# MichSchli/RelationPrediction

Measured on NVIDIA H100. Metric: R-GCN layer fwd+bwd M-edges/sec, higher is better.
Workload: dtype f32

## Files before the change

relationprediction_b200/csrc/gemm_tf32x3.cu:

```cuda
#include <cuda_runtime.h>
#include <stdint.h>

#include <algorithm>
#include <cstdlib>

#include "kernels.cuh"

namespace {

constexpr int BM = 128, BN = 128, BK = 32;
constexpr int STAGES = 3;
constexpr int TILE_BYTES = BM * BK * 4;
constexpr int STAGE_BYTES = 4 * TILE_BYTES;
constexpr int SMEM_BYTES = STAGES * STAGE_BYTES + 1024;
constexpr int N_PRODUCERS = 128;
constexpr int N_CONSUMERS = 256;
constexpr int N_THREADS = N_PRODUCERS + N_CONSUMERS;
constexpr int N_FRAG = BN / 2;
static_assert(BM == BN, "the producers use one row schedule for both operands");

__device__ __forceinline__ uint32_t smem_u32(const void* p) {
  return (uint32_t)__cvta_generic_to_shared(p);
}
__device__ __forceinline__ void mbar_init(uint64_t* bar, uint32_t count) {
  asm volatile("mbarrier.init.shared::cta.b64 [%0], %1;" ::"r"(smem_u32(bar)), "r"(count));
}
__device__ __forceinline__ void mbar_arrive(uint64_t* bar) {
  asm volatile("mbarrier.arrive.shared::cta.b64 _, [%0];" ::"r"(smem_u32(bar)) : "memory");
}
__device__ __forceinline__ void mbar_wait(uint64_t* bar, uint32_t parity) {
  asm volatile(
      "{\n\t"
      ".reg .pred p;\n\t"
      "WAIT_LOOP:\n\t"
      "mbarrier.try_wait.parity.shared::cta.b64 p, [%0], %1;\n\t"
      "@p bra WAIT_DONE;\n\t"
      "bra WAIT_LOOP;\n\t"
      "WAIT_DONE:\n\t"
      "}" ::"r"(smem_u32(bar)),
      "r"(parity)
      : "memory");
}
__device__ __forceinline__ void cp_async16(uint32_t dst, const void* src, uint32_t src_bytes) {
  asm volatile("cp.async.cg.shared.global [%0], [%1], 16, %2;" ::"r"(dst), "l"(src), "r"(src_bytes)
               : "memory");
}

__device__ __forceinline__ uint64_t make_desc(uint32_t smem_addr) {
  return (uint64_t)((smem_addr & 0x3FFFFu) >> 4) | (1ull << 16) | ((uint64_t)(1024 >> 4) << 32) | (1ull << 62);
}

__device__ __forceinline__ void wgmma_tf32(float (&d)[N_FRAG], uint64_t da, uint64_t db, uint32_t accumulate) {
  asm volatile(
      "{\n\t"
      ".reg .pred p;\n\t"
      "setp.ne.b32 p, %66, 0;\n\t"
      "wgmma.mma_async.sync.aligned.m64n128k8.f32.tf32.tf32 "
      "{%0, %1, %2, %3, %4, %5, %6, %7, %8, %9, %10, %11, %12, %13, %14, %15, %16, %17, %18, %19, %20, %21, %22, "
      "%23, %24, %25, %26, %27, %28, %29, %30, %31, %32, %33, %34, %35, %36, %37, %38, %39, %40, %41, %42, %43, %44, "
      "%45, %46, %47, %48, %49, %50, %51, %52, %53, %54, %55, %56, %57, %58, %59, %60, %61, %62, %63}, "
      "%64, %65, p, 1, 1;\n\t"
      "}"
      : "+f"(d[0]), "+f"(d[1]), "+f"(d[2]), "+f"(d[3]), "+f"(d[4]), "+f"(d[5]), "+f"(d[6]), "+f"(d[7]),
        "+f"(d[8]), "+f"(d[9]), "+f"(d[10]), "+f"(d[11]), "+f"(d[12]), "+f"(d[13]), "+f"(d[14]), "+f"(d[15]),
        "+f"(d[16]), "+f"(d[17]), "+f"(d[18]), "+f"(d[19]), "+f"(d[20]), "+f"(d[21]), "+f"(d[22]), "+f"(d[23]),
        "+f"(d[24]), "+f"(d[25]), "+f"(d[26]), "+f"(d[27]), "+f"(d[28]), "+f"(d[29]), "+f"(d[30]), "+f"(d[31]),
        "+f"(d[32]), "+f"(d[33]), "+f"(d[34]), "+f"(d[35]), "+f"(d[36]), "+f"(d[37]), "+f"(d[38]), "+f"(d[39]),
        "+f"(d[40]), "+f"(d[41]), "+f"(d[42]), "+f"(d[43]), "+f"(d[44]), "+f"(d[45]), "+f"(d[46]), "+f"(d[47]),
        "+f"(d[48]), "+f"(d[49]), "+f"(d[50]), "+f"(d[51]), "+f"(d[52]), "+f"(d[53]), "+f"(d[54]), "+f"(d[55]),
        "+f"(d[56]), "+f"(d[57]), "+f"(d[58]), "+f"(d[59]), "+f"(d[60]), "+f"(d[61]), "+f"(d[62]), "+f"(d[63])
      : "l"(da), "l"(db), "r"(accumulate)
      : "memory");
}
__device__ __forceinline__ void fence_acc(float (&d)[N_FRAG]) {
#pragma unroll
  for (int i = 0; i < N_FRAG; ++i) asm volatile("" : "+f"(d[i])::"memory");
}

__device__ __forceinline__ void split_tf32_trunc(float a, float& hi, float& lo) {
  hi = __uint_as_float(__float_as_uint(a) & 0xffffe000u);
  lo = __uint_as_float(__float_as_uint(a - hi) & 0xffffe000u);
}
__device__ __forceinline__ void split_tf32(float a, float& hi, float& lo) {
  uint32_t h, l;
  asm("cvt.rna.tf32.f32 %0, %1;" : "=r"(h) : "f"(a));
  hi = __uint_as_float(h);
  asm("cvt.rna.tf32.f32 %0, %1;" : "=r"(l) : "f"(a - hi));
  lo = __uint_as_float(l);
}

__device__ __forceinline__ uint32_t swz(int r, int c) {
  return (uint32_t)((r >> 3) * 1024 + (r & 7) * 128 + ((c ^ (r & 7)) << 4));
}

__device__ __forceinline__ void init_barriers(uint64_t* full_bar, uint64_t* empty_bar) {
  for (int s = 0; s < STAGES; ++s) {
    mbar_init(&full_bar[s], N_PRODUCERS);
    mbar_init(&empty_bar[s], N_CONSUMERS);
  }
  asm volatile("fence.mbarrier_init.release.cluster;" ::: "memory");
}

__device__ __forceinline__ void consume_tile(uint32_t smem_base, uint64_t* full_bar, uint64_t* empty_bar, int g0,
                                             int num_kb, uint32_t a_rows, float (&big)[N_FRAG],
                                             float (&small)[N_FRAG]) {
  for (int kb = 0; kb < num_kb; ++kb) {
    const int g = g0 + kb;
    const int s = g % STAGES;
    mbar_wait(&full_bar[s], (uint32_t)(g / STAGES) & 1u);
    const uint32_t a_hi = smem_base + s * STAGE_BYTES + a_rows, a_lo = a_hi + TILE_BYTES;
    const uint32_t b_hi = smem_base + s * STAGE_BYTES + 2 * TILE_BYTES, b_lo = b_hi + TILE_BYTES;
    asm volatile("wgmma.fence.sync.aligned;" ::: "memory");
#pragma unroll
    for (int kk = 0; kk < BK / 8; ++kk) {
      const uint64_t dah = make_desc(a_hi + kk * 32), dal = make_desc(a_lo + kk * 32);
      const uint64_t dbh = make_desc(b_hi + kk * 32), dbl = make_desc(b_lo + kk * 32);
      const uint32_t acc = (kb == 0 && kk == 0) ? 0u : 1u;
      wgmma_tf32(small, dal, dbh, acc);
      wgmma_tf32(small, dah, dbl, 1u);
      wgmma_tf32(big, dah, dbh, acc);
    }
    asm volatile("wgmma.commit_group.sync.aligned;" ::: "memory");
    asm volatile("wgmma.wait_group.sync.aligned 0;" ::: "memory");
    fence_acc(big);
    fence_acc(small);
    mbar_arrive(&empty_bar[s]);
  }
}

struct RankEpi {
  const float* gold_sig;
  const int32_t* gold_col;
  const uint32_t* known;
  int words;
  int32_t* raw_cnt;
  int32_t* known_cnt;
};
__device__ __forceinline__ float sigmoid_ref(float x) { return 1.0f / (1.0f + expf(-x)); }

template <int EPI>
__global__ void __launch_bounds__(N_THREADS, 1)
    k_gemm_tf32x3(const float* __restrict__ A, int64_t lda, const float* __restrict__ Bhi,
                  const float* __restrict__ Blo, int64_t ldb, float* __restrict__ C, int64_t ldc,
                  int M, int N, int K, int accumulate, int n_tiles, RankEpi re) {
  extern __shared__ uint8_t smem_raw[];
  __shared__ __align__(8) uint64_t full_bar[STAGES], empty_bar[STAGES];

  const uint32_t smem_base = (smem_u32(smem_raw) + 1023u) & ~1023u;
  const int tid = threadIdx.x, lane = tid & 31;
  const int tn = (N + BN - 1) / BN;
  const int num_kb = (K + BK - 1) / BK;
  const int n_mine = (n_tiles - (int)blockIdx.x + (int)gridDim.x - 1) / (int)gridDim.x;
  const int total_g = n_mine * num_kb;

  if (tid == 0) init_barriers(full_bar, empty_bar);
  __syncthreads();

  if (tid < N_PRODUCERS) {
    const int c = tid & 7;
    const int rbase = tid >> 3;
    const uint32_t soff = swz(rbase, c);
    constexpr int NR = BM / 16;

    int b_kb = 0, b_tile = (int)blockIdx.x, b_stage = 0;
    size_t b_off = 0;
    uint32_t b_ok = 0;
    auto b_set_tile = [&]() {
      const int r0 = (b_tile % tn) * BN + rbase;
      b_ok = 0;
#pragma unroll
      for (int i = 0; i < NR; ++i) b_ok |= (r0 + 16 * i < N ? 1u : 0u) << i;
      b_off = (b_ok & 1u) ? (size_t)r0 * ldb + c * 4 : 0;
    };
    b_set_tile();
    auto issue_b = [&]() {
      const uint32_t b_hi = smem_base + b_stage * STAGE_BYTES + 2 * TILE_BYTES + soff, b_lo = b_hi + TILE_BYTES;
      const bool col_ok = b_kb * BK + c * 4 < K;
      const size_t kof = b_off + (size_t)b_kb * BK;
#pragma unroll
      for (int i = 0; i < NR; ++i) {
        const bool ok = col_ok && ((b_ok >> i) & 1u);
        const size_t o = kof + (size_t)(16 * i) * ldb;
        cp_async16(b_hi + 2048 * i, ok ? Bhi + o : Bhi, ok ? 16u : 0u);
        cp_async16(b_lo + 2048 * i, ok ? Blo + o : Blo, ok ? 16u : 0u);
      }
      asm volatile("cp.async.commit_group;" ::: "memory");
      b_stage = b_stage + 1 == STAGES ? 0 : b_stage + 1;
      if (++b_kb == num_kb) {
        b_kb = 0;
        b_tile += (int)gridDim.x;
        b_set_tile();
      }
    };
    int a_kb = 0, a_tile = (int)blockIdx.x;
    size_t a_off = 0;
    uint32_t a_ok = 0;
    auto a_set_tile = [&]() {
      const int r0 = (a_tile / tn) * BM + rbase;
      a_ok = 0;
#pragma unroll
      for (int i = 0; i < NR; ++i) a_ok |= (r0 + 16 * i < M ? 1u : 0u) << i;
      a_off = (a_ok & 1u) ? (size_t)r0 * lda + c * 4 : 0;
    };
    a_set_tile();
    auto load_a = [&](float4 (&v)[NR]) {
      const bool col_ok = a_kb * BK + c * 4 < K;
      const float* p = A + a_off + (size_t)a_kb * BK;
#pragma unroll
      for (int i = 0; i < NR; ++i)
        v[i] = (col_ok && ((a_ok >> i) & 1u)) ? __ldg(reinterpret_cast<const float4*>(p + (size_t)(16 * i) * lda))
                                               : make_float4(0.f, 0.f, 0.f, 0.f);
      if (++a_kb == num_kb) {
        a_kb = 0;
        a_tile += (int)gridDim.x;
        a_set_tile();
      }
    };
    constexpr int PF = 2;
    float4 vbuf[PF + 1][NR];
    mbar_wait(&empty_bar[0], 1u);
    issue_b();
    for (int p = 0; p < PF; ++p)
      if (p < total_g) load_a(vbuf[p]);
    int s = 0;
    uint32_t ph_next = 0;
    for (int g0 = 0; g0 < total_g; g0 += PF + 1) {
#pragma unroll
      for (int u = 0; u <= PF; ++u) {
        const int g = g0 + u;
        if (g >= total_g) break;
        const bool more = g + 1 < total_g;
        const int s1 = s + 1 == STAGES ? 0 : s + 1;
        if (s1 == 0) ph_next ^= 1u;
        if (more) {
          mbar_wait(&empty_bar[s1], ph_next ^ 1u);
          issue_b();
        }
        if (g + PF < total_g) load_a(vbuf[(u + PF) % (PF + 1)]);
        const uint32_t a_hi = smem_base + s * STAGE_BYTES + soff, a_lo = a_hi + TILE_BYTES;
#pragma unroll
        for (int i = 0; i < NR; ++i) {
          float4 hi, lo;
          split_tf32_trunc(vbuf[u][i].x, hi.x, lo.x);
          split_tf32_trunc(vbuf[u][i].y, hi.y, lo.y);
          split_tf32_trunc(vbuf[u][i].z, hi.z, lo.z);
          split_tf32_trunc(vbuf[u][i].w, hi.w, lo.w);
          asm volatile("st.shared.v4.f32 [%0], {%1, %2, %3, %4};" ::"r"(a_hi + 2048 * i), "f"(hi.x), "f"(hi.y),
                       "f"(hi.z), "f"(hi.w)
                       : "memory");
          asm volatile("st.shared.v4.f32 [%0], {%1, %2, %3, %4};" ::"r"(a_lo + 2048 * i), "f"(lo.x), "f"(lo.y),
                       "f"(lo.z), "f"(lo.w)
                       : "memory");
        }
        if (more)
          asm volatile("cp.async.wait_group 1;" ::: "memory");
        else
          asm volatile("cp.async.wait_group 0;" ::: "memory");
        asm volatile("fence.proxy.async.shared::cta;" ::: "memory");
        mbar_arrive(&full_bar[s]);
        s = s1;
      }
    }
  } else {
    const int ctid = tid - N_PRODUCERS;
    const int wg = ctid >> 7;
    const uint32_t a_rows = (uint32_t)(wg * 64 * 128);
    float big[N_FRAG], small[N_FRAG];
    for (int ti = 0; ti < n_mine; ++ti) {
      const int tile = (int)blockIdx.x + ti * (int)gridDim.x;
      const int m0 = (tile / tn) * BM, n0 = (tile % tn) * BN;
      consume_tile(smem_base, full_bar, empty_bar, ti * num_kb, num_kb, a_rows, big, small);
      const int r0 = m0 + wg * 64 + ((ctid >> 5) & 3) * 16 + (lane >> 2);
      const int c0 = n0 + 2 * (lane & 3);
#pragma unroll
      for (int h = 0; h < 2; ++h) {
        const int row = r0 + 8 * h;
        if (EPI == 1) {
          int raw = 0, kn = 0;
          if (row < M) {
            const float gold_s = __ldg(re.gold_sig + row);
            const int gold_c = __ldg(re.gold_col + row);
#pragma unroll
            for (int cb = 0; cb < BN / 32; ++cb) {
              const int chunk = n0 + 32 * cb;
              const uint32_t kw =
                  (re.known && chunk < N) ? __ldg(re.known + (size_t)row * re.words + (chunk >> 5)) : 0u;
#pragma unroll
              for (int jj = 0; jj < 4; ++jj) {
                const int j = 4 * cb + jj;
#pragma unroll
                for (int e = 0; e < 2; ++e) {
                  const int col = c0 + 8 * j + e;
                  const float v = big[4 * j + 2 * h + e] + small[4 * j + 2 * h + e];
                  if (col < N && (sigmoid_ref(v) >= gold_s || col == gold_c)) {
                    ++raw;
                    kn += (int)((kw >> (col & 31)) & 1u);
                  }
                }
              }
            }
          }
          raw += __shfl_xor_sync(0xffffffffu, raw, 1);
          raw += __shfl_xor_sync(0xffffffffu, raw, 2);
          kn += __shfl_xor_sync(0xffffffffu, kn, 1);
          kn += __shfl_xor_sync(0xffffffffu, kn, 2);
          if ((lane & 3) == 0 && row < M) {
            if (raw) atomicAdd(re.raw_cnt + row, raw);
            if (kn) atomicAdd(re.known_cnt + row, kn);
          }
          continue;
        }
        if (row >= M) continue;
        float* crow = C + (size_t)row * ldc;
#pragma unroll
        for (int j = 0; j < BN / 8; ++j) {
          const int col = c0 + 8 * j;
          if (col < N) {
            float2 o = make_float2(big[4 * j + 2 * h] + small[4 * j + 2 * h],
                                   big[4 * j + 2 * h + 1] + small[4 * j + 2 * h + 1]);
            if (accumulate) {
              const float2 old = *reinterpret_cast<const float2*>(crow + col);
              o.x += old.x;
              o.y += old.y;
            }
            *reinterpret_cast<float2*>(crow + col) = o;
          }
        }
      }
    }
  }
}

__global__ void __launch_bounds__(N_THREADS, 1)
    k_gemm_tn_tf32x3(const float* __restrict__ A, int64_t lda, const float* __restrict__ B, int64_t ldb,
                     float* __restrict__ C, int64_t ldc, int M, int N, int K, int kb_per_split) {
  extern __shared__ uint8_t smem_raw[];
  __shared__ __align__(8) uint64_t full_bar[STAGES], empty_bar[STAGES];
  const uint32_t smem_base = (smem_u32(smem_raw) + 1023u) & ~1023u;
  const int tid = threadIdx.x, warp = tid >> 5, lane = tid & 31;
  const int m0 = blockIdx.x * BM, n0 = blockIdx.y * BN;
  const int kb_total = (K + BK - 1) / BK;
  const int kb_begin = blockIdx.z * kb_per_split;
  const int num_kb = min(kb_per_split, kb_total - kb_begin);
  if (num_kb <= 0) return;

  if (tid == 0) init_barriers(full_bar, empty_bar);
  __syncthreads();

  if (tid < N_PRODUCERS) {
    constexpr int NC = 8;
    const int kr = (lane & 15) + 16 * (warp & 1);
    const int cm0 = (lane >> 4) + 16 * (warp >> 1);
    auto load_ab = [&](int kbi, float4 (&va)[NC], float4 (&vb)[NC]) {
      const int krow = (kb_begin + kbi) * BK + kr;
      const bool kok = krow < K;
      const float* pa = A + (size_t)(kok ? krow : 0) * lda + m0;
      const float* pb = B + (size_t)(kok ? krow : 0) * ldb + n0;
#pragma unroll
      for (int i = 0; i < NC; ++i) {
        const int cm = cm0 + 2 * i;
        va[i] = (kok && m0 + 4 * cm < M) ? __ldg(reinterpret_cast<const float4*>(pa + 4 * cm))
                                         : make_float4(0.f, 0.f, 0.f, 0.f);
        vb[i] = (kok && n0 + 4 * cm < N) ? __ldg(reinterpret_cast<const float4*>(pb + 4 * cm))
                                         : make_float4(0.f, 0.f, 0.f, 0.f);
      }
    };
    auto store4 = [&](uint32_t hi_base, const float4& v, int cm) {
      const float x[4] = {v.x, v.y, v.z, v.w};
#pragma unroll
      for (int j = 0; j < 4; ++j) {
        const int r = 4 * cm + j;
        const uint32_t off =
            (uint32_t)((r >> 3) * 1024 + (r & 7) * 128 + ((((kr >> 2) ^ (r & 7)) << 4) | ((kr & 3) << 2)));
        float hi, lo;
        split_tf32_trunc(x[j], hi, lo);
        asm volatile("st.shared.f32 [%0], %1;" ::"r"(hi_base + off), "f"(hi) : "memory");
        asm volatile("st.shared.f32 [%0], %1;" ::"r"(hi_base + TILE_BYTES + off), "f"(lo) : "memory");
      }
    };
    float4 va[2][NC], vb[2][NC];
    load_ab(0, va[0], vb[0]);
    for (int kb0 = 0; kb0 < num_kb; kb0 += 2) {
#pragma unroll
      for (int u = 0; u < 2; ++u) {
        const int kbi = kb0 + u;
        if (kbi >= num_kb) break;
        if (kbi + 1 < num_kb) load_ab(kbi + 1, va[u ^ 1], vb[u ^ 1]);
        const int s = kbi % STAGES;
        mbar_wait(&empty_bar[s], ((uint32_t)(kbi / STAGES) & 1u) ^ 1u);
        const uint32_t a_hi = smem_base + s * STAGE_BYTES, b_hi = a_hi + 2 * TILE_BYTES;
#pragma unroll
        for (int i = 0; i < NC; ++i) {
          store4(a_hi, va[u][i], cm0 + 2 * i);
          store4(b_hi, vb[u][i], cm0 + 2 * i);
        }
        asm volatile("fence.proxy.async.shared::cta;" ::: "memory");
        mbar_arrive(&full_bar[s]);
      }
    }
  } else {
    const int ctid = tid - N_PRODUCERS;
    const int wg = ctid >> 7;
    float big[N_FRAG], small[N_FRAG];
    consume_tile(smem_base, full_bar, empty_bar, 0, num_kb, (uint32_t)(wg * 64 * 128), big, small);
    const int r0 = m0 + wg * 64 + ((ctid >> 5) & 3) * 16 + (lane >> 2);
    const int c0 = n0 + 2 * (lane & 3);
#pragma unroll
    for (int h = 0; h < 2; ++h) {
      const int row = r0 + 8 * h;
      if (row >= M) continue;
      float* crow = C + (size_t)row * ldc;
#pragma unroll
      for (int j = 0; j < BN / 8; ++j) {
        const int col = c0 + 8 * j;
        if (col < N)
          asm volatile("red.global.add.v2.f32 [%0], {%1, %2};" ::"l"(crow + col),
                       "f"(big[4 * j + 2 * h] + small[4 * j + 2 * h]),
                       "f"(big[4 * j + 2 * h + 1] + small[4 * j + 2 * h + 1])
                       : "memory");
      }
    }
  }
}

__global__ void k_split_b(const float* __restrict__ B, int64_t ldb, int N, int K, int transposed,
                          float* __restrict__ hi, float* __restrict__ lo) {
  const int64_t total = (int64_t)N * K;
  for (int64_t i = blockIdx.x * (int64_t)blockDim.x + threadIdx.x; i < total;
       i += (int64_t)gridDim.x * blockDim.x) {
    const int n = (int)(i / K), k = (int)(i % K);
    const float v = transposed ? __ldg(B + (size_t)k * ldb + n) : __ldg(B + (size_t)n * ldb + k);
    float h, l;
    split_tf32(v, h, l);
    hi[i] = h;
    lo[i] = l;
  }
}

}

static int sm_count() {
  int dev = 0, sms = 132;
  cudaGetDevice(&dev);
  cudaDeviceGetAttribute(&sms, cudaDevAttrMultiProcessorCount, dev);
  return sms;
}

int launch_gemm_split_b(const float* B, int64_t ldb, int N, int K, int transposed, float* hi, float* lo,
                        cudaStream_t st) {
  const int64_t total = (int64_t)N * K;
  if (total == 0) return RGCN_OK;
  int blocks = (int)((total + 255) / 256);
  if (blocks > 132 * 8) blocks = 132 * 8;
  k_split_b<<<blocks, 256, 0, st>>>(B, ldb, N, K, transposed, hi, lo);
  ++g_rgcn_launches;
  return rgcn_check_cuda(cudaGetLastError(), "k_split_b");
}

static int64_t nt_grid_cap() {
  if (const char* e = std::getenv("RGCN_GEMM_CTAS")) return std::max<int64_t>(1, std::atoll(e));
  return sm_count();
}

int launch_gemm_tf32x3(const float* A, int64_t lda, const float* Bt_hi, const float* Bt_lo, int64_t ldb,
                       float* C, int64_t ldc, int M, int N, int K, int accumulate, cudaStream_t st) {
  if (M == 0 || N == 0) return RGCN_OK;
  if (K % 4 != 0 || N % 4 != 0 || lda % 4 != 0 || ldb % 4 != 0 || ldc % 4 != 0) {
    rgcn_set_error("gemm_tf32x3: K, N and leading dimensions must be multiples of 4");
    return RGCN_ERR_INVALID;
  }
  if (K == 0) {
    if (accumulate) return RGCN_OK;
    return rgcn_check_cuda(cudaMemset2DAsync(C, ldc * sizeof(float), 0, (size_t)N * sizeof(float), M, st), "memset(C)");
  }
  static bool attr_set = false;
  if (!attr_set) {
    int rc = rgcn_check_cuda(cudaFuncSetAttribute(k_gemm_tf32x3<0>, cudaFuncAttributeMaxDynamicSharedMemorySize,
                                                  SMEM_BYTES),
                             "cudaFuncSetAttribute(gemm smem)");
    if (rc) return rc;
    attr_set = true;
  }
  const int64_t tiles = (int64_t)((M + BM - 1) / BM) * ((N + BN - 1) / BN);
  if (tiles > 0x7fffffffLL) {
    rgcn_set_error("gemm_tf32x3: too many tiles");
    return RGCN_ERR_INVALID;
  }
  dim3 grid((unsigned)std::min<int64_t>(tiles, nt_grid_cap()));
  k_gemm_tf32x3<0><<<grid, N_THREADS, SMEM_BYTES, st>>>(A, lda, Bt_hi, Bt_lo, ldb, C, ldc, M, N, K, accumulate,
                                                         (int)tiles, RankEpi{});
  ++g_rgcn_launches;
  return rgcn_check_cuda(cudaGetLastError(), "k_gemm_tf32x3");
}

int launch_gemm_rank_tf32x3(const float* Q, int64_t ldq, const float* Bt_hi, const float* Bt_lo, int64_t ldb, int M,
                            int N, int K, const float* gold_sig, const int32_t* gold_col, const uint32_t* known,
                            int words, int32_t* raw_cnt, int32_t* known_cnt, cudaStream_t st) {
  if (M == 0 || N == 0) return RGCN_OK;
  if (K <= 0 || K % 4 != 0 || ldq % 4 != 0 || ldb % 4 != 0) {
    rgcn_set_error("gemm_rank_tf32x3: K > 0; K and leading dimensions must be multiples of 4");
    return RGCN_ERR_INVALID;
  }
  static bool attr_set = false;
  if (!attr_set) {
    int rc = rgcn_check_cuda(cudaFuncSetAttribute(k_gemm_tf32x3<1>, cudaFuncAttributeMaxDynamicSharedMemorySize,
                                                  SMEM_BYTES),
                             "cudaFuncSetAttribute(gemm rank smem)");
    if (rc) return rc;
    attr_set = true;
  }
  RankEpi re{gold_sig, gold_col, known, words, raw_cnt, known_cnt};
  const int64_t tiles = (int64_t)((M + BM - 1) / BM) * ((N + BN - 1) / BN);
  if (tiles > 0x7fffffffLL) {
    rgcn_set_error("gemm_rank_tf32x3: too many tiles");
    return RGCN_ERR_INVALID;
  }
  dim3 grid((unsigned)std::min<int64_t>(tiles, nt_grid_cap()));
  k_gemm_tf32x3<1><<<grid, N_THREADS, SMEM_BYTES, st>>>(Q, ldq, Bt_hi, Bt_lo, ldb, nullptr, 0, M, N, K, 0,
                                                         (int)tiles, re);
  ++g_rgcn_launches;
  return rgcn_check_cuda(cudaGetLastError(), "k_gemm_tf32x3<rank>");
}

int launch_gemm_tn_tf32x3(const float* A, int64_t lda, const float* B, int64_t ldb, float* C, int64_t ldc,
                          int M, int N, int K, int accumulate, cudaStream_t st) {
  if (M == 0 || N == 0) return RGCN_OK;
  if (M % 4 != 0 || N % 4 != 0 || lda % 4 != 0 || ldb % 4 != 0 || ldc % 4 != 0) {
    rgcn_set_error("gemm_tn_tf32x3: M, N and leading dimensions must be multiples of 4");
    return RGCN_ERR_INVALID;
  }
  if (!accumulate) {
    int rc = rgcn_check_cuda(cudaMemset2DAsync(C, ldc * sizeof(float), 0, (size_t)N * sizeof(float), M, st),
                             "memset(C)");
    if (rc) return rc;
  }
  if (K == 0) return RGCN_OK;
  static bool attr_set = false;
  if (!attr_set) {
    int rc = rgcn_check_cuda(cudaFuncSetAttribute(k_gemm_tn_tf32x3, cudaFuncAttributeMaxDynamicSharedMemorySize,
                                                  SMEM_BYTES),
                             "cudaFuncSetAttribute(gemm tn smem)");
    if (rc) return rc;
    attr_set = true;
  }
  const int tm = (M + BM - 1) / BM, tn = (N + BN - 1) / BN;
  const int kb_total = (K + BK - 1) / BK;
  int splits = (2 * sm_count() + tm * tn - 1) / (tm * tn);
  if (splits > kb_total / 4) splits = kb_total / 4;
  if (splits < 1) splits = 1;
  const int kb_per_split = (kb_total + splits - 1) / splits;
  splits = (kb_total + kb_per_split - 1) / kb_per_split;
  dim3 grid(tm, tn, splits);
  k_gemm_tn_tf32x3<<<grid, N_THREADS, SMEM_BYTES, st>>>(A, lda, B, ldb, C, ldc, M, N, K, kb_per_split);
  ++g_rgcn_launches;
  return rgcn_check_cuda(cudaGetLastError(), "k_gemm_tn_tf32x3");
}
```

Before: 97.94.

## Stage TN GEMM operands via cp.async raw buffers and rework split-K scheduling

The producer warps now stream raw A/B tiles into a triple-buffered shared-memory staging area with cp.async. They then convert them to the swizzled hi/lo TF32 planes using vectorized shared loads and stores, replacing the earlier per-thread global-load and scalar-store path. The grid moves to a 1D tile/split layout, and a cost model picks the split-K count from wave quantization plus a fixed per-tile overhead. Consumers flush partial sums every 32 k-blocks with red.global. This aims to hide global latency and cut shared-store instruction count, at the cost of fewer conversion stages (2 instead of 3) and more atomic traffic.

```diff
diff --git a/relationprediction_b200/csrc/gemm_tf32x3.cu b/relationprediction_b200/csrc/gemm_tf32x3.cu
--- a/relationprediction_b200/csrc/gemm_tf32x3.cu
+++ b/relationprediction_b200/csrc/gemm_tf32x3.cu
@@ -93,21 +93,23 @@
   return (uint32_t)((r >> 3) * 1024 + (r & 7) * 128 + ((c ^ (r & 7)) << 4));
 }
 
+template <int NST = STAGES>
 __device__ __forceinline__ void init_barriers(uint64_t* full_bar, uint64_t* empty_bar) {
-  for (int s = 0; s < STAGES; ++s) {
+  for (int s = 0; s < NST; ++s) {
     mbar_init(&full_bar[s], N_PRODUCERS);
     mbar_init(&empty_bar[s], N_CONSUMERS);
   }
   asm volatile("fence.mbarrier_init.release.cluster;" ::: "memory");
 }
 
+template <int NST = STAGES>
 __device__ __forceinline__ void consume_tile(uint32_t smem_base, uint64_t* full_bar, uint64_t* empty_bar, int g0,
                                              int num_kb, uint32_t a_rows, float (&big)[N_FRAG],
                                              float (&small)[N_FRAG]) {
   for (int kb = 0; kb < num_kb; ++kb) {
     const int g = g0 + kb;
-    const int s = g % STAGES;
-    mbar_wait(&full_bar[s], (uint32_t)(g / STAGES) & 1u);
+    const int s = g % NST;
+    mbar_wait(&full_bar[s], (uint32_t)(g / NST) & 1u);
     const uint32_t a_hi = smem_base + s * STAGE_BYTES + a_rows, a_lo = a_hi + TILE_BYTES;
     const uint32_t b_hi = smem_base + s * STAGE_BYTES + 2 * TILE_BYTES, b_lo = b_hi + TILE_BYTES;
     asm volatile("wgmma.fence.sync.aligned;" ::: "memory");
@@ -331,93 +333,124 @@
   }
 }
 
+constexpr int TN_FLUSH_KB = 32;
+constexpr int TN_STAGES = 2;
+constexpr int TN_RAW = 3;
+constexpr int RAW_TILE_BYTES = BK * BM * 4;
+constexpr int RAW_BYTES = 2 * RAW_TILE_BYTES;
+constexpr int TN_SMEM_BYTES = TN_STAGES * STAGE_BYTES + TN_RAW * RAW_BYTES + 1024;
+static_assert(TN_SMEM_BYTES <= 227 * 1024, "TN kernel exceeds the shared memory of a block");
+static_assert(N_PRODUCERS == 128 && BK == 32 && BM == 128, "the TN producer's lane mapping assumes these");
+
+__device__ __forceinline__ float4 ld_shared_v4(uint32_t addr) {
+  float4 v;
+  asm volatile("ld.shared.v4.f32 {%0, %1, %2, %3}, [%4];" : "=f"(v.x), "=f"(v.y), "=f"(v.z), "=f"(v.w) : "r"(addr)
+               : "memory");
+  return v;
+}
+__device__ __forceinline__ void st_shared_v4(uint32_t addr, float x, float y, float z, float w) {
+  asm volatile("st.shared.v4.f32 [%0], {%1, %2, %3, %4};" ::"r"(addr), "f"(x), "f"(y), "f"(z), "f"(w) : "memory");
+}
+
 __global__ void __launch_bounds__(N_THREADS, 1)
     k_gemm_tn_tf32x3(const float* __restrict__ A, int64_t lda, const float* __restrict__ B, int64_t ldb,
                      float* __restrict__ C, int64_t ldc, int M, int N, int K, int kb_per_split) {
   extern __shared__ uint8_t smem_raw[];
-  __shared__ __align__(8) uint64_t full_bar[STAGES], empty_bar[STAGES];
+  __shared__ __align__(8) uint64_t full_bar[TN_STAGES], empty_bar[TN_STAGES];
   const uint32_t smem_base = (smem_u32(smem_raw) + 1023u) & ~1023u;
   const int tid = threadIdx.x, warp = tid >> 5, lane = tid & 31;
-  const int m0 = blockIdx.x * BM, n0 = blockIdx.y * BN;
-  const int kb_total = (K + BK - 1) / BK;
-  const int kb_begin = blockIdx.z * kb_per_split;
-  const int num_kb = min(kb_per_split, kb_total - kb_begin);
-  if (num_kb <= 0) return;
-
-  if (tid == 0) init_barriers(full_bar, empty_bar);
+  const int tm = (M + BM - 1) / BM, tiles = tm * ((N + BN - 1) / BN);
+  const int tile = (int)blockIdx.x % tiles, split = (int)blockIdx.x / tiles;
+  const int m0 = (tile % tm) * BM, n0 = (tile / tm) * BN;
+  const int kb_begin = split * kb_per_split;
+  const int num_kb = min(kb_per_split, (K + BK - 1) / BK - kb_begin);
+
+  if (tid == 0) init_barriers<TN_STAGES>(full_bar, empty_bar);
   __syncthreads();
 
   if (tid < N_PRODUCERS) {
-    constexpr int NC = 8;
-    const int kr = (lane & 15) + 16 * (warp & 1);
-    const int cm0 = (lane >> 4) + 16 * (warp >> 1);
-    auto load_ab = [&](int kbi, float4 (&va)[NC], float4 (&vb)[NC]) {
-      const int krow = (kb_begin + kbi) * BK + kr;
-      const bool kok = krow < K;
-      const float* pa = A + (size_t)(kok ? krow : 0) * lda + m0;
-      const float* pb = B + (size_t)(kok ? krow : 0) * ldb + n0;
-#pragma unroll
-      for (int i = 0; i < NC; ++i) {
-        const int cm = cm0 + 2 * i;
-        va[i] = (kok && m0 + 4 * cm < M) ? __ldg(reinterpret_cast<const float4*>(pa + 4 * cm))
-                                         : make_float4(0.f, 0.f, 0.f, 0.f);
-        vb[i] = (kok && n0 + 4 * cm < N) ? __ldg(reinterpret_cast<const float4*>(pb + 4 * cm))
-                                         : make_float4(0.f, 0.f, 0.f, 0.f);
-      }
+    const uint32_t raw_base = smem_base + TN_STAGES * STAGE_BYTES;
+    const bool a_ok = m0 + 4 * lane < M, b_ok = n0 + 4 * lane < N;
+    const float* pa = A + (a_ok ? m0 + 4 * lane : 0);
+    const float* pb = B + (b_ok ? n0 + 4 * lane : 0);
+    auto issue = [&](int kbi) {
+      const uint32_t dst = raw_base + (kbi % TN_RAW) * RAW_BYTES;
+      const int k0 = (kb_begin + kbi) * BK + warp;
+#pragma unroll
+      for (int i = 0; i < 8; ++i) {
+        const bool kok = k0 + 4 * i < K;
+        const size_t row = kok ? (size_t)(k0 + 4 * i) : 0;
+        const uint32_t off = (uint32_t)((warp + 4 * i) * 512 + ((lane ^ i) << 4));
+        cp_async16(dst + off, pa + row * lda, kok && a_ok ? 16u : 0u);
+        cp_async16(dst + RAW_TILE_BYTES + off, pb + row * ldb, kok && b_ok ? 16u : 0u);
+      }
+      asm volatile("cp.async.commit_group;" ::: "memory");
     };
-    auto store4 = [&](uint32_t hi_base, const float4& v, int cm) {
-      const float x[4] = {v.x, v.y, v.z, v.w};
-#pragma unroll
-      for (int j = 0; j < 4; ++j) {
-        const int r = 4 * cm + j;
-        const uint32_t off =
-            (uint32_t)((r >> 3) * 1024 + (r & 7) * 128 + ((((kr >> 2) ^ (r & 7)) << 4) | ((kr & 3) << 2)));
-        float hi, lo;
-        split_tf32_trunc(x[j], hi, lo);
-        asm volatile("st.shared.f32 [%0], %1;" ::"r"(hi_base + off), "f"(hi) : "memory");
-        asm volatile("st.shared.f32 [%0], %1;" ::"r"(hi_base + TILE_BYTES + off), "f"(lo) : "memory");
+    const int g = lane & 7;
+    auto convert = [&](uint32_t raw, uint32_t hi_plane) {
+#pragma unroll
+      for (int u = 0; u < 2; ++u) {
+        const int h = (lane >> 3) + 4 * warp + 16 * u;
+        float4 v[4];
+#pragma unroll
+        for (int j = 0; j < 4; ++j) v[j] = ld_shared_v4(raw + (4 * g + j) * 512 + ((h ^ g) << 4));
+        const float x[4][4] = {{v[0].x, v[1].x, v[2].x, v[3].x}, {v[0].y, v[1].y, v[2].y, v[3].y},
+                               {v[0].z, v[1].z, v[2].z, v[3].z}, {v[0].w, v[1].w, v[2].w, v[3].w}};
+#pragma unroll
+        for (int i = 0; i < 4; ++i) {
+          float hi[4], lo[4];
+#pragma unroll
+          for (int j = 0; j < 4; ++j) split_tf32_trunc(x[i][j], hi[j], lo[j]);
+          const uint32_t a = hi_plane + swz(4 * h + i, g);
+          st_shared_v4(a, hi[0], hi[1], hi[2], hi[3]);
+          st_shared_v4(a + TILE_BYTES, lo[0], lo[1], lo[2], lo[3]);
+        }
       }
     };
-    float4 va[2][NC], vb[2][NC];
-    load_ab(0, va[0], vb[0]);
-    for (int kb0 = 0; kb0 < num_kb; kb0 += 2) {
-#pragma unroll
-      for (int u = 0; u < 2; ++u) {
-        const int kbi = kb0 + u;
-        if (kbi >= num_kb) break;
-        if (kbi + 1 < num_kb) load_ab(kbi + 1, va[u ^ 1], vb[u ^ 1]);
-        const int s = kbi % STAGES;
-        mbar_wait(&empty_bar[s], ((uint32_t)(kbi / STAGES) & 1u) ^ 1u);
-        const uint32_t a_hi = smem_base + s * STAGE_BYTES, b_hi = a_hi + 2 * TILE_BYTES;
-#pragma unroll
-        for (int i = 0; i < NC; ++i) {
-          store4(a_hi, va[u][i], cm0 + 2 * i);
-          store4(b_hi, vb[u][i], cm0 + 2 * i);
-        }
-        asm volatile("fence.proxy.async.shared::cta;" ::: "memory");
-        mbar_arrive(&full_bar[s]);
-      }
+    issue(0);
+    if (num_kb > 1)
+      issue(1);
+    else
+      asm volatile("cp.async.commit_group;" ::: "memory");
+    for (int kb = 0; kb < num_kb; ++kb) {
+      asm volatile("cp.async.wait_group 1;" ::: "memory");
+      asm volatile("bar.sync 1, %0;" ::"n"(N_PRODUCERS) : "memory");
+      if (kb + 2 < num_kb)
+        issue(kb + 2);
+      else
+        asm volatile("cp.async.commit_group;" ::: "memory");
+      const int s = kb % TN_STAGES;
+      mbar_wait(&empty_bar[s], ((uint32_t)(kb / TN_STAGES) & 1u) ^ 1u);
+      const uint32_t raw = raw_base + (kb % TN_RAW) * RAW_BYTES, stage = smem_base + s * STAGE_BYTES;
+      convert(raw, stage);
+      convert(raw + RAW_TILE_BYTES, stage + 2 * TILE_BYTES);
+      asm volatile("fence.proxy.async.shared::cta;" ::: "memory");
+      mbar_arrive(&full_bar[s]);
     }
   } else {
     const int ctid = tid - N_PRODUCERS;
     const int wg = ctid >> 7;
-    float big[N_FRAG], small[N_FRAG];
-    consume_tile(smem_base, full_bar, empty_bar, 0, num_kb, (uint32_t)(wg * 64 * 128), big, small);
     const int r0 = m0 + wg * 64 + ((ctid >> 5) & 3) * 16 + (lane >> 2);
     const int c0 = n0 + 2 * (lane & 3);
-#pragma unroll
-    for (int h = 0; h < 2; ++h) {
-      const int row = r0 + 8 * h;
-      if (row >= M) continue;
-      float* crow = C + (size_t)row * ldc;
-#pragma unroll
-      for (int j = 0; j < BN / 8; ++j) {
-        const int col = c0 + 8 * j;
-        if (col < N)
-          asm volatile("red.global.add.v2.f32 [%0], {%1, %2};" ::"l"(crow + col),
-                       "f"(big[4 * j + 2 * h] + small[4 * j + 2 * h]),
-                       "f"(big[4 * j + 2 * h + 1] + small[4 * j + 2 * h + 1])
-                       : "memory");
+    float* const cbase = C + (size_t)r0 * ldc + c0;
+    float big[N_FRAG], small[N_FRAG];
+    for (int kc = 0; kc < num_kb; kc += TN_FLUSH_KB) {
+      consume_tile<TN_STAGES>(smem_base, full_bar, empty_bar, kc, min(TN_FLUSH_KB, num_kb - kc),
+                              (uint32_t)(wg * 64 * 128), big, small);
+      float* cp = cbase;
+      asm volatile("" : "+l"(cp));
+#pragma unroll
+      for (int h = 0; h < 2; ++h) {
+        if (r0 + 8 * h >= M) continue;
+        float* crow = cp + (size_t)(8 * h) * ldc;
+#pragma unroll
+        for (int j = 0; j < BN / 8; ++j) {
+          if (c0 + 8 * j < N)
+            asm volatile("red.global.add.v2.f32 [%0], {%1, %2};" ::"l"(crow + 8 * j),
+                         "f"(big[4 * j + 2 * h] + small[4 * j + 2 * h]),
+                         "f"(big[4 * j + 2 * h + 1] + small[4 * j + 2 * h + 1])
+                         : "memory");
+        }
       }
     }
   }
@@ -538,20 +571,30 @@
   static bool attr_set = false;
   if (!attr_set) {
     int rc = rgcn_check_cuda(cudaFuncSetAttribute(k_gemm_tn_tf32x3, cudaFuncAttributeMaxDynamicSharedMemorySize,
-                                                  SMEM_BYTES),
+                                                  TN_SMEM_BYTES),
                              "cudaFuncSetAttribute(gemm tn smem)");
     if (rc) return rc;
     attr_set = true;
   }
-  const int tm = (M + BM - 1) / BM, tn = (N + BN - 1) / BN;
-  const int kb_total = (K + BK - 1) / BK;
-  int splits = (2 * sm_count() + tm * tn - 1) / (tm * tn);
-  if (splits > kb_total / 4) splits = kb_total / 4;
-  if (splits < 1) splits = 1;
-  const int kb_per_split = (kb_total + splits - 1) / splits;
-  splits = (kb_total + kb_per_split - 1) / kb_per_split;
-  dim3 grid(tm, tn, splits);
-  k_gemm_tn_tf32x3<<<grid, N_THREADS, SMEM_BYTES, st>>>(A, lda, B, ldb, C, ldc, M, N, K, kb_per_split);
+  constexpr int64_t TN_KB_FIXED = 4;
+  const int64_t tiles = (int64_t)((M + BM - 1) / BM) * ((N + BN - 1) / BN);
+  const int64_t kb_total = (K + BK - 1) / BK, sms = sm_count();
+  int64_t splits = 1, kb_per_split = kb_total, best = -1;
+  for (int64_t s = 1; s <= kb_total && (s == 1 || s * tiles <= 8 * sms); ++s) {
+    const int64_t kps = (kb_total + s - 1) / s, s_eff = (kb_total + kps - 1) / kps;
+    const int64_t cost = (s_eff * tiles + sms - 1) / sms * (kps + TN_KB_FIXED);
+    if (best < 0 || cost < best) {
+      best = cost;
+      splits = s_eff;
+      kb_per_split = kps;
+    }
+  }
+  if (tiles * splits > 0x7fffffffLL) {
+    rgcn_set_error("gemm_tn_tf32x3: too many tiles");
+    return RGCN_ERR_INVALID;
+  }
+  k_gemm_tn_tf32x3<<<(unsigned)(tiles * splits), N_THREADS, TN_SMEM_BYTES, st>>>(A, lda, B, ldb, C, ldc, M, N, K,
+                                                                                 (int)kb_per_split);
   ++g_rgcn_launches;
   return rgcn_check_cuda(cudaGetLastError(), "k_gemm_tn_tf32x3");
 }
```

Result: faster. 106.3 (median of 6 runs) (+8.5%).
